# jianing-sun/Mask-YOLO

Hardware: AMD Instinct MI355X
Metric: images/sec fwd+bwd, 224x224 Shapes batch 32, at 1 MI355X (higher is better)
Workload: dtype f32

## Files before the change

### mask-yolo_amd/csrc/mem_kernels.hip

```cpp
#include "myolo_common.h"
#include <type_traits>
#include <stdlib.h>
#include <stdarg.h>
#include <string.h>

static thread_local char g_err[512] = "";
extern "C" void myolo_set_error(const char* fmt, ...)
{
    va_list ap;
    va_start(ap, fmt);
    vsnprintf(g_err, sizeof(g_err), fmt, ap);
    va_end(ap);
}
extern "C" const char* myolo_last_error_string(void) { return g_err; }
extern "C" int myolo_version(void) { return 212; }

static MyoloOptions default_options() { MyoloOptions o = {}; o.bn_fused_tf_variance = 1; o.tn_wgs = 224; return o; }
MyoloOptions g_myolo_opt = default_options();
static int* option_slot(const char* name)
{
    static const struct { const char* n; int MyoloOptions::*m; } tab[] = {
        {"gemm_generic", &MyoloOptions::gemm_generic}, {"no_splitk", &MyoloOptions::no_splitk}, {"bf16_no256", &MyoloOptions::bf16_no256},
        {"bf16_force256", &MyoloOptions::bf16_force256}, {"bf16_no_c3", &MyoloOptions::bf16_no_c3}, {"bf16_no_loopn", &MyoloOptions::bf16_no_loopn},
        {"bf16_mask_valu", &MyoloOptions::bf16_mask_valu}, {"bf16_mask_nofin", &MyoloOptions::bf16_mask_nofin},
        {"deconv_mask_legacy", &MyoloOptions::deconv_mask_legacy}, {"crop_bf16_legacy", &MyoloOptions::crop_bf16_legacy},
        {"tune0", &MyoloOptions::tune0}, {"wino_x6", &MyoloOptions::wino_x6}, {"wino_no_bt", &MyoloOptions::wino_no_bt},
        {"wino_no_mixed", &MyoloOptions::wino_no_mixed}, {"x6_no_half_tiles", &MyoloOptions::x6_no_half_tiles},
        {"w63_legacy", &MyoloOptions::w63_legacy}, {"pw_x6_min_rows", &MyoloOptions::pw_x6_min_rows}, {"deconv_no_x6", &MyoloOptions::deconv_no_x6},
        {"pw_no_smallm", &MyoloOptions::pw_no_smallm}, {"pw_no_x6", &MyoloOptions::pw_no_x6}, {"tn_no_x6", &MyoloOptions::tn_no_x6},
        {"tn_wgs", &MyoloOptions::tn_wgs}, {"no_trunk_fusion", &MyoloOptions::no_trunk_fusion},
        {"bn_fused_tf_variance", &MyoloOptions::bn_fused_tf_variance},
    };
    if (!name) return nullptr;
    for (const auto& e : tab)
        if (strcmp(e.n, name) == 0) return &(g_myolo_opt.*(e.m));
    return nullptr;
}
extern "C" int myolo_set_option(const char* name, int value)
{
    int* s = option_slot(name);
    MYOLO_REQUIRE(s, "set_option: unknown option '%s'", name ? name : "(null)");
    *s = value;
    return MYOLO_OK;
}
extern "C" int myolo_get_option(const char* name, int* value)
{
    int* s = option_slot(name);
    MYOLO_REQUIRE(s && value, "get_option: unknown option '%s'", name ? name : "(null)");
// ... 2220 lines not shown
#pragma unroll
    for (int j = 0; j < MASK_SEL_MAXCOL; ++j) acc[j] = 0.0;
    for (int c0 = 0; c0 < NR; c0 += 256) {
        __syncthreads();
        sid[tid] = c0 + tid < NR ? ids[c0 + tid] : -1;
        __syncthreads();
        const int n = NR - c0 < 256 ? NR - c0 : 256;
        for (int i = 0; i < n; ++i) {
            if (sid[i] != k || k == 0) continue;
            const double* pr = part + (long long)(c0 + i) * (Cin + 1);
#pragma unroll
            for (int j = 0; j < MASK_SEL_MAXCOL; ++j)
                if (tid + 256 * j <= Cin) acc[j] += pr[tid + 256 * j];
        }
    }
#pragma unroll
    for (int j = 0; j < MASK_SEL_MAXCOL; ++j) {
        const int c = tid + 256 * j;
        if (c < Cin) dw[(long long)c * C + k] = (float)acc[j];
        else if (c == Cin) db[k] = (float)acc[j];
    }
}

__global__ void bce_count_kernel(const int32_t* __restrict__ ids, int NR, int* __restrict__ npos)
{
    __shared__ int red[256];
    int s = 0;
    for (int i = threadIdx.x; i < NR; i += blockDim.x) s += ids[i] > 0;
    red[threadIdx.x] = s;
    __syncthreads();
    for (int o = 128; o > 0; o >>= 1) {
        if ((int)threadIdx.x < o) red[threadIdx.x] += red[threadIdx.x + o];
        __syncthreads();
    }
    if (threadIdx.x == 0) *npos = red[0];
}

__global__ __launch_bounds__(256) void bce_kernel(const float* __restrict__ tm, const int32_t* __restrict__ ids,
                                                  const float* __restrict__ pred, const int* __restrict__ npos_p,
                                                  float lw, double* __restrict__ part, float* __restrict__ dz,
                                                  int NR, int hw, int C)
{
    __shared__ double red[256];
    const long long total = (long long)NR * hw;
    const int npos = *npos_p;
    const float invn = npos > 0 ? 1.f / ((float)npos * (float)hw) : 0.f;
    double lsum = 0;
    long long i = (long long)blockIdx.x * blockDim.x + threadIdx.x;
    const long long stride = (long long)gridDim.x * blockDim.x;
    const float eps = 1e-7f;
    for (; i < total; i += stride) {
        const int roi = (int)(i / hw);
        const int id = ids[roi];
        for (int k = 0; k < C; ++k) {
            float g = 0.f;
            if (id > 0 && k == id) {
                const float p = pred[i * C + k], t = tm[i];
                const float pc = fminf(fmaxf(p, eps), 1.f - eps);
                const float z = logf(pc / (1.f - pc));
                const float l = fmaxf(z, 0.f) - z * t + log1pf(expf(-fabsf(z)));
                lsum += (double)l;
                const bool inside = (p >= eps) && (p <= 1.f - eps);
                g = inside ? (pc - t) * invn * lw : 0.f;
            }
            dz[i * C + k] = g;
        }
    }
    red[threadIdx.x] = lsum;
// ... 3 lines not shown
        __syncthreads();
    }
    if (threadIdx.x == 0) part[blockIdx.x] = red[0];
}

__global__ __launch_bounds__(256) void bce_finish_kernel(const double* __restrict__ part, int nblk, const int* __restrict__ npos_p, int hw,
                                                         float* __restrict__ out)
{
    __shared__ double red[256];
    double s = 0;
    for (int b = threadIdx.x; b < nblk; b += 256) s += part[b];
    red[threadIdx.x] = s;
    __syncthreads();
    for (int o = 128; o > 0; o >>= 1) {
        if ((int)threadIdx.x < o) red[threadIdx.x] += red[threadIdx.x + o];
        __syncthreads();
    }
    if (threadIdx.x != 0) return;
    const int npos = *npos_p;
    out[0] = npos > 0 ? (float)(red[0] / ((double)npos * hw)) : 0.f;
    out[1] = (float)npos;
}

__global__ __launch_bounds__(256) void bce_sel_kernel(const float* __restrict__ tm, const int32_t* __restrict__ ids,
                                                      const float* __restrict__ pred, const int* __restrict__ npos_p,
                                                      float lw, double* __restrict__ part, float* __restrict__ dz_sel,
                                                      int NR, int hw, int C)
{
    __shared__ double red[256];
    const long long total = (long long)NR * hw;
    const int npos = *npos_p;
    const float invn = npos > 0 ? 1.f / ((float)npos * (float)hw) : 0.f;
    double lsum = 0;
    long long i = (long long)blockIdx.x * blockDim.x + threadIdx.x;
    const long long stride = (long long)gridDim.x * blockDim.x;
    const float eps = 1e-7f;
    for (; i < total; i += stride) {
        const int id = ids[(int)(i / hw)];
        float g = 0.f;
        if (id > 0 && id < C) {
            const float p = pred[i * C + id], t = tm[i];
            const float pc = fminf(fmaxf(p, eps), 1.f - eps);
            const float z = logf(pc / (1.f - pc));
            const float l = fmaxf(z, 0.f) - z * t + log1pf(expf(-fabsf(z)));
            lsum += (double)l;
            const bool inside = (p >= eps) && (p <= 1.f - eps);
            g = inside ? (pc - t) * invn * lw : 0.f;
        }
        dz_sel[i] = g;
    }
    red[threadIdx.x] = lsum;
    __syncthreads();
    for (int o = 128; o > 0; o >>= 1) {
        if ((int)threadIdx.x < o) red[threadIdx.x] += red[threadIdx.x + o];
// ... 969 lines not shown
                            int C, void* ws, size_t ws_bytes, void* stream)
{
    MYOLO_REQUIRE(x && w && dz && dx && dw && db && M > 0 && (Cin & 3) == 0 && C >= 1 && C <= MASK_MAXC,
                  "mask_head_out_bwd: bad arguments (1<=C<=%d; more classes: myolo_mask_head_out_bwd_sel)", MASK_MAXC);
    hipStream_t s = (hipStream_t)stream;
    int rc = MYOLO_EINVAL;
#define MO_CASE(K) case K: rc = mask_out_bwd_impl<K>(x, w, dz, dx, dw, db, M, Cin, ws, ws_bytes, s); break;
    switch (C) { MO_CASE(1) MO_CASE(2) MO_CASE(3) MO_CASE(4) MO_CASE(5) MO_CASE(6) MO_CASE(7) MO_CASE(8) }
#undef MO_CASE
    if (rc) return rc;
    MYOLO_CHECK_LAUNCH();
    return MYOLO_OK;
}

int myolo_mask_bce(const float* target_masks, const int32_t* target_class_ids, const float* pred, float loss_weight,
                   float* loss_out, float* dz, int NR, int h, int w, int C, void* ws, size_t ws_bytes, void* stream)
{
    MYOLO_REQUIRE(target_masks && target_class_ids && pred && loss_out && dz && NR > 0 && C > 0, "mask_bce: bad arguments");
    const int nblk = 1024;
    MYOLO_NEED_WS(256 + nblk * sizeof(double));
    int* npos = (int*)ws;
    double* part = (double*)((char*)ws + 256);
    hipStream_t s = (hipStream_t)stream;
    hipLaunchKernelGGL(bce_count_kernel, dim3(1), dim3(256), 0, s, target_class_ids, NR, npos);
    hipLaunchKernelGGL(bce_kernel, dim3(nblk), dim3(256), 0, s, target_masks, target_class_ids, pred, npos, loss_weight, part, dz,
                       NR, h * w, C);
    hipLaunchKernelGGL(bce_finish_kernel, dim3(1), dim3(256), 0, s, part, nblk, npos, h * w, loss_out);
    MYOLO_CHECK_LAUNCH();
    return MYOLO_OK;
}

int myolo_mask_bce_sel(const float* target_masks, const int32_t* target_class_ids, const float* pred, float loss_weight,
                       float* loss_out, float* dz_sel, int NR, int h, int w, int C, void* ws, size_t ws_bytes, void* stream)
{
    MYOLO_REQUIRE(target_masks && target_class_ids && pred && loss_out && dz_sel && NR > 0 && C > 0, "mask_bce_sel: bad arguments");
    const int nblk = 1024;
    MYOLO_NEED_WS(256 + nblk * sizeof(double));
    int* npos = (int*)ws;
    double* part = (double*)((char*)ws + 256);
    hipStream_t s = (hipStream_t)stream;
    hipLaunchKernelGGL(bce_count_kernel, dim3(1), dim3(256), 0, s, target_class_ids, NR, npos);
    hipLaunchKernelGGL(bce_sel_kernel, dim3(nblk), dim3(256), 0, s, target_masks, target_class_ids, pred, npos, loss_weight, part, dz_sel,
                       NR, h * w, C);
    hipLaunchKernelGGL(bce_finish_kernel, dim3(1), dim3(256), 0, s, part, nblk, npos, h * w, loss_out);
    MYOLO_CHECK_LAUNCH();
    return MYOLO_OK;
}

size_t myolo_mask_head_out_bwd_sel_ws_bytes(int NR, int Cin)
{
    return NR > 0 && Cin > 0 ? (size_t)NR * (Cin + 1) * sizeof(double) : 0;
}

int myolo_mask_head_out_bwd_sel(const float* x, const float* w, const float* dz_sel, const int32_t* ids, float* dx, float* dw, float* db,
                                int64_t M, int Cin, int C, int hw, void* ws, size_t ws_bytes, void* stream)
{
    MYOLO_REQUIRE(x && w && dz_sel && ids && dx && dw && db && M > 0 && C >= 1 && hw > 0 && M % hw == 0 && M / hw <= 0x7fffffff,
                  "mask_head_out_bwd_sel: bad arguments");
    MYOLO_REQUIRE((Cin & 3) == 0 && Cin > 0 && 256 % (Cin >> 2) == 0 && Cin + 1 <= 256 * MASK_SEL_MAXCOL,
                  "mask_head_out_bwd_sel: Cin / 4 must divide 256 (got Cin %d)", Cin);
    const int NR = (int)(M / hw);
    MYOLO_NEED_WS(myolo_mask_head_out_bwd_sel_ws_bytes(NR, Cin));
    double* part = (double*)ws;
    hipStream_t s = (hipStream_t)stream;
    hipLaunchKernelGGL(mask_out_bwd_sel_kernel, dim3((unsigned)NR), dim3(256), 0, s, x, w, dz_sel, ids, dx, part, Cin, C, hw);
    hipLaunchKernelGGL(mask_out_bwd_sel_finish, dim3((unsigned)C), dim3(256), 0, s, part, ids, dw, db, NR, Cin, C);
// ... 74 lines not shown
```

### mask-yolo_amd/csrc/myolo_common.h

```cpp
#pragma once
#include <hip/hip_runtime.h>
#include <stdint.h>
#include <stdio.h>
#include "../../include/myolo_hip_internal.h"

extern "C" void myolo_set_error(const char* fmt, ...);

struct MyoloOptions {
    int gemm_generic;
    int no_splitk;
    int bf16_no256;
    int bf16_no_loopn;
    int bf16_mask_valu;
    int bf16_mask_nofin;
    int deconv_mask_legacy;
    int bf16_no_c3;
    int bf16_force256;
    int crop_bf16_legacy;
    int tune0;
    int wino_x6;
    int wino_no_bt;
    int wino_no_mixed;
    int x6_no_half_tiles;
    int w63_legacy;
    int pw_x6_min_rows;
    int deconv_no_x6;
    int pw_no_smallm;
    int pw_no_x6;
    int tn_no_x6;
    int tn_wgs;
    int no_trunk_fusion;
    int bn_fused_tf_variance;
};
extern MyoloOptions g_myolo_opt;

#define MYOLO_REQUIRE(cond, ...)                                   \
    do {                                                           \
        if (!(cond)) {                                             \
// ... 72 lines not shown
```

### mask-yolo_amd/csrc/wino63_kernels.hip

```cpp
#include "myolo_common.h"

#define W63_HW 14
#define W63_CS 64
#define W63_TILES 9

__host__ __device__ constexpr int w63_s6(int p) { return p == 7 ? 5 : p; }
__host__ __device__ constexpr int w63_q(int i, int j)
{
    const bool ci = (i == 5 || i == 6), cj = (j == 5 || j == 6);
    return !ci ? (!cj ? w63_s6(i) * 6 + w63_s6(j) : 36 + w63_s6(i) * 2 + (j - 5)) : (!cj ? 48 + (i - 5) * 6 + w63_s6(j) : 60 + (i - 5) * 2 + (j - 5));
}
__host__ __device__ constexpr int w63_grp(int i, int j) { return ((i == 5 || i == 6) ? 2 : 0) + ((j == 5 || j == 6) ? 1 : 0); }
__host__ __device__ constexpr int w63_qfirst(int g) { return g == 0 ? 0 : g == 1 ? 36 : g == 2 ? 48 : 60; }

typedef float f2 __attribute__((ext_vector_type(2)));
template <typename T> __device__ __forceinline__ T w63_zero() { return (T)(0.f); }
__device__ __forceinline__ float w63_fma(float a, float b, float c) { return __builtin_fmaf(a, b, c); }
__device__ __forceinline__ f2 w63_fma(float a, f2 b, f2 c) { const f2 av = {a, a}; return __builtin_elementwise_fma(av, b, c); }
template <int CLS, typename T = float>
__device__ __forceinline__ void w63_bt(const T d[8], T t[8])
{
#pragma clang fp contract(off)
    if (CLS == 6) {
        const T e0 = w63_fma(-4.25f, d[4], d[2] + d[6]), o0 = w63_fma(-4.25f, d[3], d[1] + d[5]);
// ... 96 lines not shown
}
#define W63_ADDR(pl, i, j) ((pl).base[w63_grp(i, j)] + (long long)(w63_q(i, j) - w63_qfirst(w63_grp(i, j))) * (pl).stride[w63_grp(i, j)])
template <int CLS>
__device__ __forceinline__ constexpr bool w63_used(int p) { return CLS == 6 || (p != 5 && p != 6); }

struct W63Args {
    const float* src;
    float* Vn;
    float* y;
    const int32_t* flags;
    const float* bias;
    const float* scale;
    const float* shift;
    long long NR;
    int C, act;
    const float* dyc;
    const int32_t* inv;
    const float* ka;
    const float* kb;
    const float* boxes;
    const int32_t* bind;
    int FH, FW;
    double* stats;
    float* Qn;
    float* ypre;
    int keep_cap;
};

__device__ __forceinline__ int w63_cload(const int32_t* p, long long i) { return ((const __attribute__((address_space(4))) int32_t*)p)[i]; }
__device__ __forceinline__ float w63_cload(const float* p, long long i) { return ((const __attribute__((address_space(4))) float*)p)[i]; }
__device__ __forceinline__ long long w63_keep_dst(const W63Args& a, long long img)
{
    if (!a.flags) return img;
    const int f = w63_cload(a.flags, img);
    if (a.keep_cap > 0) return (f >= 0 && f < a.keep_cap) ? (long long)f : -1;
    return f != 0 ? img : -1;
}

__device__ __forceinline__ float w63_act(float v, int act)
{
    if (act == MYOLO_ACT_RELU) return fmaxf(v, 0.f);
    if (act == MYOLO_ACT_RELU6) return fminf(fmaxf(v, 0.f), 6.f);
    return v;
}

template <int CY, int CX, bool TO_LDS>
// ... 469 lines not shown
    constexpr int LDS_TILE = BACK == W63_TO_NONE ? 2 * W63_TILES * W63_CS : W63_HW * W63_HW * W63_CS;
    float pf[64];
    int slot = -1;
#define W63Q_ISSUE_ACT(IMG)                                                                                                          \
    do {                                                                                                                             \
        const __amdgpu_buffer_rsrc_t rx = w63_rsrc(a.src + ((long long)(IMG) * W63_HW * W63_HW) * a.C + c0, img_bytes);              \
        _Pragma("unroll") for (int k = 0; k < W63_NPW; ++k)                                                                          \
            pf[k] = w63_ld(rx, lane4, (unsigned)min(wave + k * W63_TILES, W63_HW * W63_HW - 1) * C * 4u);                             \
        if (FRONT == W63_FROM_LAZY) {                                                                                                \
            slot = w63_cload(a.inv, (IMG));                                                                                          \
            if (slot >= 0) {                                                                                                         \
                const __amdgpu_buffer_rsrc_t rg = w63_rsrc(a.dyc + ((long long)slot * W63_HW * W63_HW) * a.C + c0, img_bytes);       \
                _Pragma("unroll") for (int k = 0; k < W63_NPW; ++k)                                                                  \
                    pf[32 + k] = w63_ld(rg, lane4, (unsigned)min(wave + k * W63_TILES, W63_HW * W63_HW - 1) * C * 4u);                \
            }                                                                                                                        \
        }                                                                                                                            \
    } while (0)
    if (unit < nunits) {
        const unsigned img = unit / ns;
        if (FRONT == W63_FROM_M) w63q_issue_m<CY, CX>(pf, rsrc, w63p_planes(NR, img, ty, tx, C, c0), lane4);
        else if (FRONT == W63_FROM_ACT || FRONT == W63_FROM_LAZY) W63Q_ISSUE_ACT(img);
    }
    int buf = 0;
#ifdef W63_TRACE
    int w63_it = -1;
#endif
    for (; unit < nunits; unit += stride, buf ^= 1) {
#ifdef W63_TRACE
        ++w63_it;
#endif
        W63_T(0);
        const unsigned img = unit / ns;
        const unsigned nxt = unit + stride;
        const bool more = nxt < nunits;
        const unsigned nimg = nxt / ns;
        float* act = lds + buf * LDS_TILE;
        const W63U pl = w63p_planes(NR, img, ty, tx, C, c0);
        if (FRONT == W63_FROM_M) {
            W63Keep kp;
            const long long yd = a.ypre ? (long long)img : w63_keep_dst(a, img);
            kp.wy = a.y && yd >= 0;
            kp.y = w63_rsrc(a.y + (yd * W63_HW * W63_HW) * a.C + c0, kp.wy ? img_bytes : 0u);
            const long long pd = a.ypre ? w63_keep_dst(a, img) : -1;
            kp.wp = pd >= 0;
            kp.p = w63_rsrc(a.ypre + (pd * W63_HW * W63_HW) * a.C + c0, kp.wp ? img_bytes : 0u);
            f2 tmp[6][4];
            w63q_col_m<CY, CX>(pf, tmp);
            W63_T(1);
            if (more) w63q_issue_m<CY, CX>(pf, rsrc, w63p_planes(NR, nimg, ty, tx, C, c0), lane4);
            float s1 = 0.f, s2 = 0.f;
            w63q_row_m<CY, CX, BACK, ACT>(tmp, cb, sc, sh, kp, C, act, oy, ox, lane, s1, s2);
            if (BACK == W63_TO_NONE && a.stats) {
                act[tile * W63_CS + lane] = s1; act[(W63_TILES + tile) * W63_CS + lane] = s2;
                __syncthreads();
                if (wave == 0) {
                    double t1 = 0, t2 = 0;
#pragma unroll
                    for (int k = 0; k < W63_TILES; ++k) { t1 += (double)act[k * W63_CS + lane]; t2 += (double)act[(W63_TILES + k) * W63_CS + lane]; }
                    double* dst = a.stats + (long long)img * 2 * a.C;
                    dst[c] = t1;
                    dst[a.C + c] = t2;
                }
            }
        } else if (FRONT == W63_FROM_CROP) {
            const float by1 = w63_cload(a.boxes, (long long)img * 4), bx1 = w63_cload(a.boxes, (long long)img * 4 + 1);
            const float by2 = w63_cload(a.boxes, (long long)img * 4 + 2), bx2 = w63_cload(a.boxes, (long long)img * 4 + 3);
            const int cq = (lane & 15) * 4;
            const float* fb = a.src + (long long)w63_cload(a.bind, img) * a.FH * a.FW * a.C + c0 + cq;
            constexpr int NP = 3;
            constexpr int STEP = 4 * W63_TILES;
            for (int p0 = wave * 4 + (lane >> 4); p0 < W63_HW * W63_HW; p0 += NP * STEP) {
                float4 tl[NP], tr[NP], bl[NP], br[NP];
                float wx[NP], wy[NP];
                bool ok[NP];
#pragma unroll
                for (int k = 0; k < NP; ++k) {
                    const int pix = min(p0 + k * STEP, W63_HW * W63_HW - 1);
                    const int py = pix / W63_HW, px = pix - py * W63_HW;
                    const W63CropAxis ay = w63_crop_axis(by1, by2, a.FH, W63_HW, py), ax = w63_crop_axis(bx1, bx2, a.FW, W63_HW, px);
                    ok[k] = ay.ok && ax.ok; wx[k] = ax.w; wy[k] = ay.w;
                    tl[k] = *reinterpret_cast<const float4*>(fb + ((long long)ay.lo * a.FW + ax.lo) * a.C);
                    tr[k] = *reinterpret_cast<const float4*>(fb + ((long long)ay.lo * a.FW + ax.hi) * a.C);
                    bl[k] = *reinterpret_cast<const float4*>(fb + ((long long)ay.hi * a.FW + ax.lo) * a.C);
                    br[k] = *reinterpret_cast<const float4*>(fb + ((long long)ay.hi * a.FW + ax.hi) * a.C);
// ... 31 lines not shown
            }
            if (more) W63Q_ISSUE_ACT(nimg);
#pragma unroll
            for (int k = 0; k < W63_NPW; ++k) {
                const int pix = wave + k * W63_TILES;
                if (pix < W63_HW * W63_HW) act[pix * W63_CS + lane] = v[k];
            }
            if (wy) {
#pragma unroll
                for (int k = 0; k < W63_NPW; ++k) {
                    const int pix = wave + k * W63_TILES;
                    if (pix < W63_HW * W63_HW) w63_st(v[k], ry, lane4, (unsigned)pix * C * 4u);
                }
            }
        }
        W63_T(2);
        if (BACK == W63_TO_NONE) continue;
        __syncthreads();
        if (BACK == W63_TO_Q || BACK == W63_TO_VQ) w63p_back_q<CY, CX>(rq, pl, act, oy, ox, lane);
        W63_T(3);
        if (BACK == W63_TO_V || BACK == W63_TO_VQ) w63p_back_v<CY, CX>(rv, pl, act, py0, px0, ey, ex, lane);
        W63_T(4);
    }
#undef W63Q_ISSUE_ACT
}

template <int FRONT, int BACK, int ACT>
__global__ __launch_bounds__(W63_TILES * 64) void wino63_boundary_kernel(W63Args a)
{
    extern __shared__ __attribute__((aligned(16))) float act_lds[];
    const int lane = threadIdx.x & 63, wave = __builtin_amdgcn_readfirstlane(threadIdx.x >> 6);
    const int ty = wave / 3, tx = wave - ty * 3;
    if (ty == 0) { if (tx == 0) w63q_loop<6, 6, FRONT, BACK, ACT>(a, act_lds, ty, tx, wave, lane); else w63q_loop<6, 4, FRONT, BACK, ACT>(a, act_lds, ty, tx, wave, lane); }
    else         { if (tx == 0) w63q_loop<4, 6, FRONT, BACK, ACT>(a, act_lds, ty, tx, wave, lane); else w63q_loop<4, 4, FRONT, BACK, ACT>(a, act_lds, ty, tx, wave, lane); }
}


__global__ __launch_bounds__(256) void wino63_dw_kernel(const float* __restrict__ dU, float* __restrict__ dw, int Ci, int Co)
{
    const int idx = blockIdx.x * blockDim.x + threadIdx.x;
    if (idx >= Ci * Co) return;
    const long long plane = (long long)Ci * Co;
    float tmp[3][8];
#pragma unroll
    for (int j = 0; j < 8; ++j) {
        float col[8], r[3];
// ... 57 lines not shown
static int w63_layout(int K, int N) { return myolo_gemm_nt_batched_x6(K, N) ? 2 : 1; }

static int w63_num_cus()
{
    static int n = 0;
    if (!n) {
        int dev = 0;
        hipDeviceProp_t prop;
        if (hipGetDevice(&dev) != hipSuccess || hipGetDeviceProperties(&prop, dev) != hipSuccess || prop.multiProcessorCount <= 0) return 256;
        n = prop.multiProcessorCount;
    }
    return n;
}
template <int FRONT, int BACK, int ACT>
static void w63_launch_act(const W63Args& b, unsigned grid, size_t lds, hipStream_t s)
{
    static bool attr_set = false;
    if (!attr_set) {
        (void)hipFuncSetAttribute((const void*)wino63_boundary_kernel<FRONT, BACK, ACT>, hipFuncAttributeMaxDynamicSharedMemorySize, (int)lds);
        attr_set = true;
    }
    hipLaunchKernelGGL((wino63_boundary_kernel<FRONT, BACK, ACT>), dim3(grid), dim3(W63_TILES * 64), lds, s, b);
}
template <int FRONT, int BACK>
static int w63_launch(const W63Args& a, hipStream_t s)
{
    const long long units = a.NR * (a.C / W63_CS);
    if (units <= 0 || units >= (1LL << 31)) return MYOLO_EINVAL;
    const bool one_unit = g_myolo_opt.w63_legacy || FRONT == W63_FROM_CROP || (unsigned long long)400 * a.NR * a.C * 4ull >= (1ull << 32);
    if (one_unit) {
        static bool attr_set = false;
        const size_t lds = (size_t)W63_HW * W63_HW * W63_CS * sizeof(float);
        if (!attr_set) {
            (void)hipFuncSetAttribute((const void*)wino63_boundary_legacy_kernel<FRONT, BACK>, hipFuncAttributeMaxDynamicSharedMemorySize, (int)lds);
            attr_set = true;
        }
        hipLaunchKernelGGL((wino63_boundary_legacy_kernel<FRONT, BACK>), dim3((unsigned)units), dim3(W63_TILES * 64), lds, s, a);
        return MYOLO_OK;
    }
    const int ns = a.C / W63_CS;
    long long grid = w63_num_cus();
    grid -= grid % ns;
    if (grid < ns) grid = ns;
    if (grid > units) grid = units;
    const size_t lds = 2 * sizeof(float) * (BACK == W63_TO_NONE ? (size_t)2 * W63_TILES * W63_CS : (size_t)W63_HW * W63_HW * W63_CS);
    if (FRONT == W63_FROM_LAZY || FRONT == W63_FROM_CROP || a.act == MYOLO_ACT_NONE) w63_launch_act<FRONT, BACK, MYOLO_ACT_NONE>(a, (unsigned)grid, lds, s);
    else if (a.act == MYOLO_ACT_RELU) w63_launch_act<FRONT, BACK, MYOLO_ACT_RELU>(a, (unsigned)grid, lds, s);
    else w63_launch_act<FRONT, BACK, MYOLO_ACT_RELU6>(a, (unsigned)grid, lds, s);
    return MYOLO_OK;
}

extern "C" {

int myolo_wino63_ok(int H, int W, int Cin, int Cout)
{
    return H == W63_HW && W == W63_HW && (Cin % W63_CS) == 0 && (Cout % W63_CS) == 0 && myolo_gemm_nt_batched_ok(Cin, Cout) ? 1 : 0;
}
size_t myolo_wino63_plane_elems(int N, int C) { return (size_t)400 * (size_t)N * (size_t)C; }
size_t myolo_wino63_u_elems(int Cin, int Cout) { return align256((size_t)64 * Cin * Cout * 6) / sizeof(float); }

int myolo_wino63_weight_transform(const float* w, float* U, int Cin, int Cout, void* stream)
{
    MYOLO_REQUIRE(w && U && myolo_wino63_ok(W63_HW, W63_HW, Cin, Cout), "wino63_weight_transform: needs Cin, Cout multiples of 64 with Cin %% 16 == 0, Cout %% 256 == 0 (got %d, %d)", Cin, Cout);
    hipLaunchKernelGGL(wino63_w_kernel, dim3((Cin * Cout + 255) / 256), dim3(256), 0, (hipStream_t)stream, w, U, Cin, Cout, w63_layout(Cin, Cout), 0);
    MYOLO_CHECK_LAUNCH();
    return MYOLO_OK;
}
// ... 107 lines not shown

int myolo_wino63_output_transform(const float* M, const float* bias, const float* scale, const float* shift, float* y, int N, int C, int act,
                                  void* stream)
{
    MYOLO_REQUIRE(M && y && N > 0 && (C % W63_CS) == 0 && !scale == !shift, "wino63_output_transform: bad arguments (C %% 64 == 0)");
    W63Args a{M, nullptr, y, nullptr, bias, scale, shift, N, C, act};
    w63_launch<W63_FROM_M, W63_TO_NONE>(a, (hipStream_t)stream);
    MYOLO_CHECK_LAUNCH();
    return MYOLO_OK;
}

int myolo_wino63_input_transform_roialign(const float* feature, const float* boxes, const int32_t* box_ind, float* V, int B, int FH, int FW,
                                          int C, int nb, void* stream)
{
    MYOLO_REQUIRE(feature && boxes && box_ind && V && B > 0 && FH > 0 && FW > 0 && nb > 0 && (C % W63_CS) == 0,
                  "wino63_input_transform_roialign: bad arguments (C %% 64 == 0)");
    W63Args a{};
    a.src = feature; a.Vn = V; a.NR = nb; a.C = C; a.act = MYOLO_ACT_NONE; a.boxes = boxes; a.bind = box_ind; a.FH = FH; a.FW = FW;
    w63_launch<W63_FROM_CROP, W63_TO_V>(a, (hipStream_t)stream);
    MYOLO_CHECK_LAUNCH();
    return MYOLO_OK;
}

size_t myolo_wino63_output_transform_bn_ws_bytes(int N, int C) { return align256((size_t)N * 2 * C * sizeof(double)) + 2 * C * sizeof(double); }

int myolo_wino63_output_transform_bn_stats(const float* M, const float* bias, float* y, int N, int C, const float* gamma, const float* beta,
                                           float* mean, float* var, float* scale, float* shift, float* moving_mean, float* moving_var,
                                           void* ws, size_t ws_bytes, void* stream)
{
    MYOLO_REQUIRE(M && y && gamma && beta && mean && var && scale && shift && N > 0 && (C % W63_CS) == 0, "wino63_output_transform_bn_stats: bad arguments");
    MYOLO_NEED_WS(myolo_wino63_output_transform_bn_ws_bytes(N, C));
    hipStream_t s = (hipStream_t)stream;
    double* part = (double*)ws;
    double* tot = (double*)((char*)ws + align256((size_t)N * 2 * C * sizeof(double)));
    W63Args a{};
    a.src = M; a.y = y; a.bias = bias; a.NR = N; a.C = C; a.act = MYOLO_ACT_NONE; a.stats = part;
    w63_launch<W63_FROM_M, W63_TO_NONE>(a, s);
    myolo_bn_stats_from_partials(part, tot, N, C, (double)N * W63_HW * W63_HW, gamma, beta, mean, var, scale, shift, moving_mean, moving_var, s);
    MYOLO_CHECK_LAUNCH();
    return MYOLO_OK;
}

#ifdef W63_TRACE
int myolo_w63_trace_read(void* dst, size_t bytes) { return hipMemcpyFromSymbol(dst, HIP_SYMBOL(w63_trace_buf), bytes) == hipSuccess ? 0 : -1; }
#endif
static const long long* w63_run_rows(long long NR, long long rows[3]) { rows[0] = 9 * NR; rows[1] = 3 * NR; rows[2] = NR; return rows; }

}

static int w63_tn_and_dw(const float* V, const float* Q, float* dU, float* dw, int N, int Cin, int Cout, void* part, size_t part_bytes, hipStream_t s)
{
    long long rows[3];
    w63_run_rows(N, rows);
    const int nq[3] = {36, 24, 4};
    const long long prow[3] = {0, 36 * rows[0], 36 * rows[0] + 24 * rows[1]};
    const long long pq[3] = {0, 36, 60};
    if (myolo_gemm_tn_x6_ok(Cin, Cout)) {
        const long long ao[3] = {prow[0] * Cin, prow[1] * Cin, prow[2] * Cin}, bo[3] = {prow[0] * Cout, prow[1] * Cout, prow[2] * Cout};
        const int rc = myolo_gemm_tn_x6_runs(V, Q, dU, 3, rows, ao, bo, nq, Cin, Cout, part, part_bytes, s);
        if (rc != MYOLO_OK) return rc;
        hipLaunchKernelGGL(wino63_dw_kernel, dim3((Cin * Cout + 255) / 256), dim3(256), 0, s, dU, dw, Cin, Cout);
// ... 196 lines not shown
```

### mask-yolo_amd/myolo/engine.py

```python
import contextlib
import os
import threading
import time

import numpy as np
import torch

from . import _ext as X

ACT_NONE, ACT_RELU, ACT_RELU6 = 0, 1, 2

BACKBONE_BLOCKS = [(64, 1), (64, 2), (128, 1), (256, 2), (256, 1), (512, 1)]
YOLO_BLOCKS = [(512, 2), (512, 1), (512, 1), (512, 1), (512, 1), (512, 1), (1024, 2), (1024, 1)]
MASK_FILTERS = 256
RESNET_STAGES = [(2, "abc", (64, 64, 256), 1), (3, "abcd", (128, 128, 512), 2), (4, "abcdef", (256, 256, 1024), 2), (5, "abc", (512, 512, 2048), 2)]
RESNET_C4_STAGE = 3
RESNET_MAX_MASK_ROIS = 32 * 7 * 7 * 3


def resnet_check_size(n_images, h, w, n_box):
    rois = int(n_images) * (int(h) // 32) * (int(w) // 32) * int(n_box)
    if rois > RESNET_MAX_MASK_ROIS:
        raise ValueError("BACKBONE='resnet50': %d images of %dx%d with N_BOX=%d give %d mask-head ROIs per launch; only up to %d are supported "
                         "(larger launches have not been audited against the kernels' 32-bit buffer descriptors)"
# ... 193 lines not shown
                    items = [("gamma", (shp,)), ("beta", (shp,))]
                    for s in ("moving_mean", "moving_variance"):
                        self.sslots[name + "/" + s] = (soff, (shp,))
                        soff += shp
                for s, sh in items:
                    n = int(np.prod(sh))
                    self.pslots[name + "/" + s] = (off, tuple(sh))
                    off += (n + 3) // 4 * 4
            self.bucket_ranges.append((b0, off))
        self.nparam = off
        f32 = dict(dtype=torch.float32, device=self.dev)
        self.flat_p = torch.zeros(off, **f32)
        self.flat_g = torch.zeros(off, **f32)
        self.flat_m = torch.zeros(off, **f32)
        self.flat_v = torch.zeros(off, **f32)
        self.flat_s = torch.zeros(soff, **f32)
        self.p = {k: self.flat_p[o:o + int(np.prod(sh))].view(sh) for k, (o, sh) in self.pslots.items()}
        self.g = {k: self.flat_g[o:o + int(np.prod(sh))].view(sh) for k, (o, sh) in self.pslots.items()}
        self.s = {k: self.flat_s[o:o + int(np.prod(sh))].view(sh) for k, (o, sh) in self.sslots.items()}
        self.bnbuf = {}
        for name, kind, shp, _ in self.table:
            if kind == "bn":
                self.bnbuf[name] = torch.zeros(4, shp, **f32)
        self._graphs = {}
        self._lanes = {}
        self._cap_stream = None
        self._fm_stream = None
        self.infer_fork_feature_map = False
        self._fork_now = None
        self._ws_main = Workspace(self.dev, on_realloc=lambda: self._drop_graphs(0))
        self._side = None
        self._yolo_stream = _shared_stream(self.dev, "yolo_head_bwd")
        self._yolo_side = _Side(self._yolo_stream, Workspace(self.dev))
        self.yolo_bwd_early = -1
        self.exchange_active = False
        self._wgrad_stream = _shared_stream(self.dev, "weight_gradients")
        self._wgrad_side = _Side(self._wgrad_stream, Workspace(self.dev))
        self._twg_stream = self._wgrad_stream
        self.lazy_bn1_bwd = True
        self.fold_frozen_bn = True
        self.fuse_trunk_bn = bool(getattr(cfg, "FUSE_TRUNK_BN", True))
        self._fz_table = None
        self.anchors = torch.tensor(np.asarray(cfg.ANCHORS, np.float32), device=self.dev)
        self.class_weights = torch.tensor(np.asarray(cfg.CLASS_WEIGHTS, np.float32), device=self.dev)
        self.adam_t = 0
        self.tape = {}
# ... 278 lines not shown
        elif self._wino_ok(nimg, h, w, cout, cin):
            self.ws.ensure(X.wino_ws_bytes(nimg, h, w, cin, cout, 1))
            X.call("myolo_conv3x3_wino_bwd_data", X.ptr(dy), X.ptr(self.p[layer + "/kernel"]), X.ptr(dx), nimg, h, w, cin, cout,
                   *self._wsargs(), X.stream())
        else:
            X.call("myolo_conv3x3_bwd_data", X.ptr(dy), X.ptr(self.p[layer + "/kernel"]), X.ptr(dx), nimg, h, w, cin, cout,
                   *self._wsargs(), X.stream())

    def _frozen_affine_all(self):
        if self._fz_table is None:
            rows, off = [], 0
            self._fz_slot = {}
            for name in sorted(k[:-len("/gamma")] for k in self.pslots if self._trunk_bn(k)):
                C = int(self.p[name + "/gamma"].numel())
                rows.append([self.pslots[name + "/gamma"][0], self.pslots[name + "/beta"][0], self.sslots[name + "/moving_mean"][0],
                             self.sslots[name + "/moving_variance"][0], off, C])
                self._fz_slot[name] = (off, C)
                off += 2 * C
            self._fz_table = torch.tensor(rows, dtype=torch.int64, device=self.dev)
            self._fz_coeffs = torch.empty(off, dtype=torch.float32, device=self.dev)
        X.call("myolo_bn_frozen_coeffs_batched", X.ptr(self.flat_p), X.ptr(self.flat_s), self._fz_table.data_ptr(), int(self._fz_table.shape[0]),
               X.ptr(self._fz_coeffs), X.stream())

    def _trunk_bn(self, key):
        if not key.endswith("/gamma"):
            return False
        if self.resnet:
            return key.startswith("bn_conv1/") or (key.startswith("bn") and key[2:3].isdigit())
        return key.endswith("_bn/gamma") and (key.startswith("conv_dw_") or key.startswith("conv_pw_") or key.startswith("conv1_bn/"))

    def _frozen_affine(self, name):
        off, C = self._fz_slot[name]
        base = self._fz_coeffs.data_ptr()
        return base + 4 * off, base + 4 * (off + C)

    @staticmethod
    def _is_lazy(a):
        return isinstance(a, tuple) and a[0] == "lazy"

    def _in_args(self, a):
        if self._is_lazy(a):
            _, y, bn = a
            buf = self.bnbuf[bn]
            return X.ptr(y), X.ptr(buf[2]), X.ptr(buf[3]), ACT_RELU6
        return X.ptr(a), None, None, ACT_NONE

# ... 478 lines not shown
                X.call("myolo_deconv2x2s2_mask_fwd_keep", X.ptr(x), X.ptr(self.p["myolo_mask_deconv/kernel"]),
                       X.ptr(self.p["myolo_mask_deconv/bias"]), X.ptr(self.p["myolo_mask/kernel"]), X.ptr(self.p["myolo_mask/bias"]),
                       X.ptr(p), NR, ps, ps, MASK_FILTERS, MASK_FILTERS, C, X.ptr(inv_d), X.ptr(dk), cap, *self._wsargs(), X.stream())
                d = ("kept", dk, cap)
            else:
                X.call("myolo_deconv2x2s2_mask_fwd", X.ptr(x), X.ptr(self.p["myolo_mask_deconv/kernel"]),
                       X.ptr(self.p["myolo_mask_deconv/bias"]), X.ptr(self.p["myolo_mask/kernel"]), X.ptr(self.p["myolo_mask/bias"]),
                       X.ptr(p), NR, ps, ps, MASK_FILTERS, MASK_FILTERS, C, *self._wsargs(), X.stream())
        else:
            d = self._new(NR * 4 * ps * ps, MASK_FILTERS)
            X.call("myolo_deconv2x2s2_fwd", X.ptr(x), X.ptr(self.p["myolo_mask_deconv/kernel"]), X.ptr(self.p["myolo_mask_deconv/bias"]),
                   X.ptr(d), NR, ps, ps, MASK_FILTERS, MASK_FILTERS, ACT_RELU, *self._wsargs(), X.stream())
            X.call("myolo_mask_head_out_fwd", X.ptr(d), X.ptr(self.p["myolo_mask/kernel"]), X.ptr(self.p["myolo_mask/bias"]), X.ptr(p),
                   NR * 4 * ps * ps, MASK_FILTERS, C, X.stream())
        self.tape["mask"] = (convs, x, d)
        return p

    def _mask_convs_winograd_chain(self, x, convs, NR, ps, cin, train, pos_flags, roi=None, slots=None):
        q = ps * ps
        Vcur = None
        t63 = self.wino_tiles == "f63" and X.wino63_ok(ps, ps, MASK_FILTERS, MASK_FILTERS)
        c1_63 = (t63 and X.wino63_ok(ps, ps, cin, MASK_FILTERS) and X.wino63_ok(ps, ps, MASK_FILTERS, cin)
                 and (not train or (self.lazy_bn1_bwd and self.sparse_mask_bwd)))
        for i in range(1, 5):
            cn, bn = "myolo_mask_conv%d" % i, "myolo_mask_bn%d" % i
            batch_stats = train and i == 1
            fold = not batch_stats
            use63 = t63 and (i >= 2 or c1_63)
            next63 = t63 and i < 4
            T = NR * ((ps + 3) // 4) ** 2
            start, stop = self._timed("mask_conv3x3_fwd")
            start()
            if Vcur is None:
                if use63:
                    Vcur = self._new(X.wino63_plane_elems(NR, cin))
                    if x is None:
                        Fm, boxes, bind, fn, fh, fw = roi
                        self._call_timed("roialign_fwd", "myolo_wino63_input_transform_roialign", X.ptr(Fm), X.ptr(boxes), X.ptr(bind),
                                         X.ptr(Vcur), fn, fh, fw, cin, NR, X.stream())
                    else:
                        self._call_timed("wino_in", "myolo_wino63_input_transform", X.ptr(x), None, None, ACT_NONE, None, None, X.ptr(Vcur),
                                         NR, cin, X.stream())
                else:
                    Vcur = self._new(36, T, cin)
                    if x is None:
                        Fm, boxes, bind, fn, fh, fw = roi
                        self._call_timed("roialign_fwd", "myolo_wino_input_transform_roialign", X.ptr(Fm), X.ptr(boxes), X.ptr(bind),
                                         X.ptr(Vcur), fn, fh, fw, cin, NR, ps, ps, X.stream())
                    else:
                        self._call_timed("wino_in", "myolo_wino_input_transform", X.ptr(x), X.ptr(Vcur), NR, ps, ps, cin, X.stream())
            if use63:
                U, M = self._new(X.wino63_u_elems(cin, MASK_FILTERS)), self._new(X.wino63_plane_elems(NR, MASK_FILTERS))
                self._call_timed("wino_multiply", "myolo_wino63_multiply_w", X.ptr(Vcur), X.ptr(self.p[cn + "/kernel"]), X.ptr(U), X.ptr(M), NR, cin,
                                 MASK_FILTERS, X.stream())
            else:
                U, M = self._new(X.wino_u_elems(cin, MASK_FILTERS)), self._new(36, T, MASK_FILTERS)
                X.call("myolo_wino_weight_transform", X.ptr(self.p[cn + "/kernel"]), X.ptr(U), cin, MASK_FILTERS, 0, X.stream())
                self._call_timed("wino_multiply", "myolo_wino_multiply", X.ptr(Vcur), X.ptr(U), X.ptr(M), NR, ps, ps, cin, MASK_FILTERS,
                                 X.stream())
            if i == 1 and train:
                self.tape["conv1_V"] = Vcur
                self.tape["conv1_V_fmt"] = "f63" if use63 else "f43"
            convs.append(x)
            bias = self.p[cn + "/bias"]
            buf = self.bnbuf[bn]
            if fold:
                X.call("myolo_bn_frozen_coeffs", X.ptr(self.p[bn + "/gamma"]), X.ptr(self.p[bn + "/beta"]),
                       X.ptr(self.s[bn + "/moving_mean"]), X.ptr(self.s[bn + "/moving_variance"]),
                       X.ptr(buf[2]), X.ptr(buf[3]), MASK_FILTERS, X.stream())
                self.tape[bn] = (None, ACT_RELU, False)
            if fold and i < 4 and use63 == next63:
                ykeep = self._new(NR * q, MASK_FILTERS) if train else None
                keep_pre = bool(train)
                if use63:
                    Vn = self._new(X.wino63_plane_elems(NR, MASK_FILTERS))
                    if keep_pre and slots is not None:
                        self._call_timed("wino_out_in", "myolo_wino63_output_input_transform_keep_pre_slots", X.ptr(M), X.ptr(bias), X.ptr(buf[2]),
                                         X.ptr(buf[3]), X.ptr(ykeep), X.ptr(slots), NR, X.ptr(Vn), NR, MASK_FILTERS, ACT_RELU, X.stream())
                        self.tape.setdefault("compact_rows", set()).add(id(ykeep))
                    elif keep_pre:
                        self._call_timed("wino_out_in", "myolo_wino63_output_input_transform_keep_pre", X.ptr(M), X.ptr(bias), X.ptr(buf[2]),
                                         X.ptr(buf[3]), X.ptr(ykeep), X.ptr(pos_flags), X.ptr(Vn), NR, MASK_FILTERS, ACT_RELU, X.stream())
                    else:
                        self._call_timed("wino_out_in", "myolo_wino63_output_input_transform", X.ptr(M), X.ptr(bias), X.ptr(buf[2]),
                                         X.ptr(buf[3]), X.ptr(ykeep), X.ptr(pos_flags) if train else None, X.ptr(Vn), NR, MASK_FILTERS,
                                         ACT_RELU, X.stream())
                else:
                    Vn = self._new(36, T, MASK_FILTERS)
                    self._call_timed("wino_out_in", "myolo_wino_output_input_transform_keep_pre" if keep_pre else "myolo_wino_output_input_transform",
                                     X.ptr(M), X.ptr(bias), X.ptr(buf[2]), X.ptr(buf[3]), X.ptr(ykeep), X.ptr(pos_flags) if train else None, X.ptr(Vn),
                                     NR, ps, ps, MASK_FILTERS, ACT_RELU, X.stream())
                if keep_pre:
# ... 1021 lines not shown
```

Measured before the change: 1665.

## Fuse BCE positive count, accumulate BN stats per workgroup, batch mask BN coeffs

Every block of the BCE and selected-BCE loss kernels now computes the positive-ROI count itself, so the separate single-block count launch is dropped. The wino63 output-transform BN-stats path accumulates per-channel sums per persistent workgroup, not per image, which shrinks the partials buffer and the later reduction. Frozen BN coefficients for mask layers 2-4 are computed with one batched call instead of three separate launches. The intent is fewer tiny kernel launches and less reduction work. The cost is that each BCE block redundantly scans the ids array, and the old paths remain behind a chain_legacy option.

```diff
diff --git a/mask-yolo_amd/csrc/mem_kernels.hip b/mask-yolo_amd/csrc/mem_kernels.hip
--- a/mask-yolo_amd/csrc/mem_kernels.hip
+++ b/mask-yolo_amd/csrc/mem_kernels.hip
@@ -23,7 +23,7 @@
         {"gemm_generic", &MyoloOptions::gemm_generic}, {"no_splitk", &MyoloOptions::no_splitk}, {"bf16_no256", &MyoloOptions::bf16_no256},
         {"bf16_force256", &MyoloOptions::bf16_force256}, {"bf16_no_c3", &MyoloOptions::bf16_no_c3}, {"bf16_no_loopn", &MyoloOptions::bf16_no_loopn},
         {"bf16_mask_valu", &MyoloOptions::bf16_mask_valu}, {"bf16_mask_nofin", &MyoloOptions::bf16_mask_nofin},
-        {"deconv_mask_legacy", &MyoloOptions::deconv_mask_legacy}, {"crop_bf16_legacy", &MyoloOptions::crop_bf16_legacy},
+        {"deconv_mask_legacy", &MyoloOptions::deconv_mask_legacy}, {"chain_legacy", &MyoloOptions::chain_legacy}, {"crop_bf16_legacy", &MyoloOptions::crop_bf16_legacy},
         {"tune0", &MyoloOptions::tune0}, {"wino_x6", &MyoloOptions::wino_x6}, {"wino_no_bt", &MyoloOptions::wino_no_bt},
         {"wino_no_mixed", &MyoloOptions::wino_no_mixed}, {"x6_no_half_tiles", &MyoloOptions::x6_no_half_tiles},
         {"w63_legacy", &MyoloOptions::w63_legacy}, {"pw_x6_min_rows", &MyoloOptions::pw_x6_min_rows}, {"deconv_no_x6", &MyoloOptions::deconv_no_x6},
@@ -2290,6 +2290,20 @@
     }
 }
 
+__device__ __forceinline__ int bce_count_block(const int32_t* __restrict__ ids, int NR)
+{
+    __shared__ int cnt[256];
+    int s = 0;
+    for (int i = threadIdx.x; i < NR; i += 256) s += ids[i] > 0;
+    cnt[threadIdx.x] = s;
+    __syncthreads();
+    for (int o = 128; o > 0; o >>= 1) {
+        if ((int)threadIdx.x < o) cnt[threadIdx.x] += cnt[threadIdx.x + o];
+        __syncthreads();
+    }
+    return cnt[0];
+}
+
 __global__ void bce_count_kernel(const int32_t* __restrict__ ids, int NR, int* __restrict__ npos)
 {
     __shared__ int red[256];
@@ -2304,14 +2318,16 @@
     if (threadIdx.x == 0) *npos = red[0];
 }
 
+template <bool COUNT>
 __global__ __launch_bounds__(256) void bce_kernel(const float* __restrict__ tm, const int32_t* __restrict__ ids,
-                                                  const float* __restrict__ pred, const int* __restrict__ npos_p,
+                                                  const float* __restrict__ pred, int* __restrict__ npos_p,
                                                   float lw, double* __restrict__ part, float* __restrict__ dz,
                                                   int NR, int hw, int C)
 {
     __shared__ double red[256];
     const long long total = (long long)NR * hw;
-    const int npos = *npos_p;
+    const int npos = COUNT ? bce_count_block(ids, NR) : *npos_p;
+    if (COUNT && blockIdx.x == 0 && threadIdx.x == 0) *npos_p = npos;
     const float invn = npos > 0 ? 1.f / ((float)npos * (float)hw) : 0.f;
     double lsum = 0;
     long long i = (long long)blockIdx.x * blockDim.x + threadIdx.x;
@@ -2361,14 +2377,16 @@
     out[1] = (float)npos;
 }
 
+template <bool COUNT>
 __global__ __launch_bounds__(256) void bce_sel_kernel(const float* __restrict__ tm, const int32_t* __restrict__ ids,
-                                                      const float* __restrict__ pred, const int* __restrict__ npos_p,
+                                                      const float* __restrict__ pred, int* __restrict__ npos_p,
                                                       float lw, double* __restrict__ part, float* __restrict__ dz_sel,
                                                       int NR, int hw, int C)
 {
     __shared__ double red[256];
     const long long total = (long long)NR * hw;
-    const int npos = *npos_p;
+    const int npos = COUNT ? bce_count_block(ids, NR) : *npos_p;
+    if (COUNT && blockIdx.x == 0 && threadIdx.x == 0) *npos_p = npos;
     const float invn = npos > 0 ? 1.f / ((float)npos * (float)hw) : 0.f;
     double lsum = 0;
     long long i = (long long)blockIdx.x * blockDim.x + threadIdx.x;
@@ -3384,9 +3402,13 @@
     int* npos = (int*)ws;
     double* part = (double*)((char*)ws + 256);
     hipStream_t s = (hipStream_t)stream;
-    hipLaunchKernelGGL(bce_count_kernel, dim3(1), dim3(256), 0, s, target_class_ids, NR, npos);
-    hipLaunchKernelGGL(bce_kernel, dim3(nblk), dim3(256), 0, s, target_masks, target_class_ids, pred, npos, loss_weight, part, dz,
-                       NR, h * w, C);
+    if (g_myolo_opt.chain_legacy) {
+        hipLaunchKernelGGL(bce_count_kernel, dim3(1), dim3(256), 0, s, target_class_ids, NR, npos);
+        hipLaunchKernelGGL((bce_kernel<false>), dim3(nblk), dim3(256), 0, s, target_masks, target_class_ids, pred, npos, loss_weight, part, dz,
+                           NR, h * w, C);
+    } else
+        hipLaunchKernelGGL((bce_kernel<true>), dim3(nblk), dim3(256), 0, s, target_masks, target_class_ids, pred, npos, loss_weight, part, dz,
+                           NR, h * w, C);
     hipLaunchKernelGGL(bce_finish_kernel, dim3(1), dim3(256), 0, s, part, nblk, npos, h * w, loss_out);
     MYOLO_CHECK_LAUNCH();
     return MYOLO_OK;
@@ -3401,9 +3423,13 @@
     int* npos = (int*)ws;
     double* part = (double*)((char*)ws + 256);
     hipStream_t s = (hipStream_t)stream;
-    hipLaunchKernelGGL(bce_count_kernel, dim3(1), dim3(256), 0, s, target_class_ids, NR, npos);
-    hipLaunchKernelGGL(bce_sel_kernel, dim3(nblk), dim3(256), 0, s, target_masks, target_class_ids, pred, npos, loss_weight, part, dz_sel,
-                       NR, h * w, C);
+    if (g_myolo_opt.chain_legacy) {
+        hipLaunchKernelGGL(bce_count_kernel, dim3(1), dim3(256), 0, s, target_class_ids, NR, npos);
+        hipLaunchKernelGGL((bce_sel_kernel<false>), dim3(nblk), dim3(256), 0, s, target_masks, target_class_ids, pred, npos, loss_weight, part, dz_sel,
+                           NR, h * w, C);
+    } else
+        hipLaunchKernelGGL((bce_sel_kernel<true>), dim3(nblk), dim3(256), 0, s, target_masks, target_class_ids, pred, npos, loss_weight, part, dz_sel,
+                           NR, h * w, C);
     hipLaunchKernelGGL(bce_finish_kernel, dim3(1), dim3(256), 0, s, part, nblk, npos, h * w, loss_out);
     MYOLO_CHECK_LAUNCH();
     return MYOLO_OK;
diff --git a/mask-yolo_amd/csrc/myolo_common.h b/mask-yolo_amd/csrc/myolo_common.h
--- a/mask-yolo_amd/csrc/myolo_common.h
+++ b/mask-yolo_amd/csrc/myolo_common.h
@@ -14,6 +14,7 @@
     int bf16_mask_valu;
     int bf16_mask_nofin;
     int deconv_mask_legacy;
+    int chain_legacy;
     int bf16_no_c3;
     int bf16_force256;
     int crop_bf16_legacy;
diff --git a/mask-yolo_amd/csrc/wino63_kernels.hip b/mask-yolo_amd/csrc/wino63_kernels.hip
--- a/mask-yolo_amd/csrc/wino63_kernels.hip
+++ b/mask-yolo_amd/csrc/wino63_kernels.hip
@@ -142,6 +142,7 @@
     const int32_t* bind;
     int FH, FW;
     double* stats;
+    int stats_wg;
     float* Qn;
     float* ypre;
     int keep_cap;
@@ -657,6 +658,7 @@
         else if (FRONT == W63_FROM_ACT || FRONT == W63_FROM_LAZY) W63Q_ISSUE_ACT(img);
     }
     int buf = 0;
+    double wg1 = 0, wg2 = 0;
 #ifdef W63_TRACE
     int w63_it = -1;
 #endif
@@ -692,9 +694,12 @@
                     double t1 = 0, t2 = 0;
 #pragma unroll
                     for (int k = 0; k < W63_TILES; ++k) { t1 += (double)act[k * W63_CS + lane]; t2 += (double)act[(W63_TILES + k) * W63_CS + lane]; }
-                    double* dst = a.stats + (long long)img * 2 * a.C;
-                    dst[c] = t1;
-                    dst[a.C + c] = t2;
+                    if (a.stats_wg) { wg1 += t1; wg2 += t2; }
+                    else {
+                        double* dst = a.stats + (long long)img * 2 * a.C;
+                        dst[c] = t1;
+                        dst[a.C + c] = t2;
+                    }
                 }
             }
         } else if (FRONT == W63_FROM_CROP) {
@@ -772,6 +777,11 @@
         if (BACK == W63_TO_V || BACK == W63_TO_VQ) w63p_back_v<CY, CX>(rv, pl, act, py0, px0, ey, ex, lane);
         W63_T(4);
     }
+    if (FRONT == W63_FROM_M && BACK == W63_TO_NONE && a.stats && a.stats_wg && wave == 0 && blockIdx.x < nunits) {
+        double* dst = a.stats + (long long)(blockIdx.x / ns) * 2 * a.C;
+        dst[c] = wg1;
+        dst[a.C + c] = wg2;
+    }
 #undef W63Q_ISSUE_ACT
 }
 
@@ -875,13 +885,29 @@
     }
     hipLaunchKernelGGL((wino63_boundary_kernel<FRONT, BACK, ACT>), dim3(grid), dim3(W63_TILES * 64), lds, s, b);
 }
+static bool w63_one_unit(long long NR, int C) { return g_myolo_opt.w63_legacy || (unsigned long long)400 * NR * C * 4ull >= (1ull << 32); }
+static long long w63_persistent_grid(long long NR, int C)
+{
+    const int ns = C / W63_CS;
+    long long grid = w63_num_cus();
+    grid -= grid % ns;
+    if (grid < ns) grid = ns;
+    if (grid > NR * ns) grid = NR * ns;
+    return grid;
+}
+static long long w63_stat_rows(long long NR, int C)
+{
+    return (w63_one_unit(NR, C) || g_myolo_opt.chain_legacy) ? NR : w63_persistent_grid(NR, C) / (C / W63_CS);
+}
+
 template <int FRONT, int BACK>
 static int w63_launch(const W63Args& a, hipStream_t s)
 {
     const long long units = a.NR * (a.C / W63_CS);
     if (units <= 0 || units >= (1LL << 31)) return MYOLO_EINVAL;
-    const bool one_unit = g_myolo_opt.w63_legacy || FRONT == W63_FROM_CROP || (unsigned long long)400 * a.NR * a.C * 4ull >= (1ull << 32);
+    const bool one_unit = FRONT == W63_FROM_CROP || w63_one_unit(a.NR, a.C);
     if (one_unit) {
+        if (a.stats && a.stats_wg) return MYOLO_EINVAL;
         static bool attr_set = false;
         const size_t lds = (size_t)W63_HW * W63_HW * W63_CS * sizeof(float);
         if (!attr_set) {
@@ -891,11 +917,7 @@
         hipLaunchKernelGGL((wino63_boundary_legacy_kernel<FRONT, BACK>), dim3((unsigned)units), dim3(W63_TILES * 64), lds, s, a);
         return MYOLO_OK;
     }
-    const int ns = a.C / W63_CS;
-    long long grid = w63_num_cus();
-    grid -= grid % ns;
-    if (grid < ns) grid = ns;
-    if (grid > units) grid = units;
+    const long long grid = w63_persistent_grid(a.NR, a.C);
     const size_t lds = 2 * sizeof(float) * (BACK == W63_TO_NONE ? (size_t)2 * W63_TILES * W63_CS : (size_t)W63_HW * W63_HW * W63_CS);
     if (FRONT == W63_FROM_LAZY || FRONT == W63_FROM_CROP || a.act == MYOLO_ACT_NONE) w63_launch_act<FRONT, BACK, MYOLO_ACT_NONE>(a, (unsigned)grid, lds, s);
     else if (a.act == MYOLO_ACT_RELU) w63_launch_act<FRONT, BACK, MYOLO_ACT_RELU>(a, (unsigned)grid, lds, s);
@@ -1049,7 +1071,11 @@
     return MYOLO_OK;
 }
 
-size_t myolo_wino63_output_transform_bn_ws_bytes(int N, int C) { return align256((size_t)N * 2 * C * sizeof(double)) + 2 * C * sizeof(double); }
+size_t myolo_wino63_output_transform_bn_ws_bytes(int N, int C)
+{
+    if (N <= 0 || C <= 0 || (C % W63_CS) != 0) return 0;
+    return align256((size_t)w63_stat_rows(N, C) * 2 * C * sizeof(double)) + 2 * C * sizeof(double);
+}
 
 int myolo_wino63_output_transform_bn_stats(const float* M, const float* bias, float* y, int N, int C, const float* gamma, const float* beta,
                                            float* mean, float* var, float* scale, float* shift, float* moving_mean, float* moving_var,
@@ -1058,12 +1084,15 @@
     MYOLO_REQUIRE(M && y && gamma && beta && mean && var && scale && shift && N > 0 && (C % W63_CS) == 0, "wino63_output_transform_bn_stats: bad arguments");
     MYOLO_NEED_WS(myolo_wino63_output_transform_bn_ws_bytes(N, C));
     hipStream_t s = (hipStream_t)stream;
+    const long long rows = w63_stat_rows(N, C);
     double* part = (double*)ws;
-    double* tot = (double*)((char*)ws + align256((size_t)N * 2 * C * sizeof(double)));
+    double* tot = (double*)((char*)ws + align256((size_t)rows * 2 * C * sizeof(double)));
     W63Args a{};
-    a.src = M; a.y = y; a.bias = bias; a.NR = N; a.C = C; a.act = MYOLO_ACT_NONE; a.stats = part;
-    w63_launch<W63_FROM_M, W63_TO_NONE>(a, s);
-    myolo_bn_stats_from_partials(part, tot, N, C, (double)N * W63_HW * W63_HW, gamma, beta, mean, var, scale, shift, moving_mean, moving_var, s);
+    a.src = M; a.y = y; a.bias = bias; a.NR = N; a.C = C; a.act = MYOLO_ACT_NONE; a.stats = part; 
+    a.stats_wg = !(w63_one_unit(N, C) || g_myolo_opt.chain_legacy);
+    const int rc = w63_launch<W63_FROM_M, W63_TO_NONE>(a, s);
+    if (rc != MYOLO_OK) { myolo_set_error("wino63_output_transform_bn_stats: bad problem size"); return rc; }
+    myolo_bn_stats_from_partials(part, tot, (int)rows, C, (double)N * W63_HW * W63_HW, gamma, beta, mean, var, scale, shift, moving_mean, moving_var, s);
     MYOLO_CHECK_LAUNCH();
     return MYOLO_OK;
 }
diff --git a/mask-yolo_amd/myolo/engine.py b/mask-yolo_amd/myolo/engine.py
--- a/mask-yolo_amd/myolo/engine.py
+++ b/mask-yolo_amd/myolo/engine.py
@@ -239,6 +239,7 @@
         for name, kind, shp, _ in self.table:
             if kind == "bn":
                 self.bnbuf[name] = torch.zeros(4, shp, **f32)
+        self._mask_fz_table = None
         self._graphs = {}
         self._lanes = {}
         self._cap_stream = None
@@ -563,6 +564,16 @@
         X.call("myolo_bn_frozen_coeffs_batched", X.ptr(self.flat_p), X.ptr(self.flat_s), self._fz_table.data_ptr(), int(self._fz_table.shape[0]),
                X.ptr(self._fz_coeffs), X.stream())
 
+    def _mask_frozen_affine(self, layers):
+        if self._mask_fz_table is None or self._mask_fz_table[0] != layers:
+            bufs = [self.bnbuf[name] for name in layers]
+            base = min(b[2].data_ptr() for b in bufs)
+            rows = [[self.pslots[name + "/gamma"][0], self.pslots[name + "/beta"][0], self.sslots[name + "/moving_mean"][0],
+                     self.sslots[name + "/moving_variance"][0], (b[2].data_ptr() - base) // 4, int(b.shape[1])] for name, b in zip(layers, bufs)]
+            self._mask_fz_table = (layers, torch.tensor(rows, dtype=torch.int64, device=self.dev), base)
+        _, table, base = self._mask_fz_table
+        X.call("myolo_bn_frozen_coeffs_batched", X.ptr(self.flat_p), X.ptr(self.flat_s), table.data_ptr(), int(table.shape[0]), base, X.stream())
+
     def _trunk_bn(self, key):
         if not key.endswith("/gamma"):
             return False
@@ -1087,6 +1098,9 @@
         t63 = self.wino_tiles == "f63" and X.wino63_ok(ps, ps, MASK_FILTERS, MASK_FILTERS)
         c1_63 = (t63 and X.wino63_ok(ps, ps, cin, MASK_FILTERS) and X.wino63_ok(ps, ps, MASK_FILTERS, cin)
                  and (not train or (self.lazy_bn1_bwd and self.sparse_mask_bwd)))
+        batched_coeffs = bool(train)
+        if batched_coeffs:
+            self._mask_frozen_affine(("myolo_mask_bn2", "myolo_mask_bn3", "myolo_mask_bn4"))
         for i in range(1, 5):
             cn, bn = "myolo_mask_conv%d" % i, "myolo_mask_bn%d" % i
             batch_stats = train and i == 1
@@ -1130,9 +1144,10 @@
             bias = self.p[cn + "/bias"]
             buf = self.bnbuf[bn]
             if fold:
-                X.call("myolo_bn_frozen_coeffs", X.ptr(self.p[bn + "/gamma"]), X.ptr(self.p[bn + "/beta"]),
-                       X.ptr(self.s[bn + "/moving_mean"]), X.ptr(self.s[bn + "/moving_variance"]),
-                       X.ptr(buf[2]), X.ptr(buf[3]), MASK_FILTERS, X.stream())
+                if not batched_coeffs:
+                    X.call("myolo_bn_frozen_coeffs", X.ptr(self.p[bn + "/gamma"]), X.ptr(self.p[bn + "/beta"]),
+                           X.ptr(self.s[bn + "/moving_mean"]), X.ptr(self.s[bn + "/moving_variance"]),
+                           X.ptr(buf[2]), X.ptr(buf[3]), MASK_FILTERS, X.stream())
                 self.tape[bn] = (None, ACT_RELU, False)
             if fold and i < 4 and use63 == next63:
                 ykeep = self._new(NR * q, MASK_FILTERS) if train else None
```

Measured after the change: 1662. About the same (-0.1%).
